# naman1618/Distributed-Inference-with-PyTorch-and-LiteLLM

Measured on AMD Instinct MI355X. Metric: fine-tune tokens/sec (whole node) Llama-3.1-70B DDP at 1/2/4/8 MI355X, higher is better.
Workload: dtype bf16; 1 GPU; model=Llama-3.1-70B, global_batch=2, seq_len=2048, parallelism=dp1, finetune=lora r=16 alpha=32.0 on q,k,v,o,gate,up,down; frozen bf16 base, micro_batch=2, grad_accum=1, activation_checkpointing=False, optimizer=fused AdamW (HIP), grad clip 1.0, grad_reduce_dtype=bf16

## Files before the change

### csrc/kernels/lora.hip

```cpp
#include "bindings.h"
#include "common.h"
#include <stdlib.h>
#include <string.h>

namespace mx {

namespace {

typedef __bf16 lbf16x8_t __attribute__((ext_vector_type(8)));
typedef __attribute__((address_space(1))) const void* lgptr_t;
typedef __attribute__((address_space(3))) void* llptr_t;

__device__ __forceinline__ f32x4 lmfma(const u16x8& a, const u16x8& b, const f32x4& c) {
  return __builtin_amdgcn_mfma_f32_16x16x32_bf16(__builtin_bit_cast(lbf16x8_t, a), __builtin_bit_cast(lbf16x8_t, b),
                                                 c, 0, 0, 0);
}

constexpr int kRS = 68;
constexpr int kMaxTiles = 16384;

__device__ unsigned int g_xwt_cnt[kMaxTiles];
__device__ unsigned int g_xtg_cnt[kMaxTiles];

__device__ __forceinline__ bool arrive_last(unsigned int* cnt, int S, int* s_flag) {
// ... 58 lines not shown
#pragma unroll
  for (int i = 0; i < 4; ++i)
#pragma unroll
    for (int j = 0; j < 4; ++j) acc[i][j] = f32x4{0.f, 0.f, 0.f, 0.f};

  auto load = [&](int b, u16x8(&xr)[4][2], u16x8(&vr)[4][2]) {
    const int k0 = b * 64;
#pragma unroll
    for (int i = 0; i < 4; ++i)
#pragma unroll
      for (int p = 0; p < 2; ++p) {
        xr[i][p] = *reinterpret_cast<const u16x8*>(xp + i * xrb + k0 + 8 * p);
        vr[i][p] = *reinterpret_cast<const u16x8*>(vp + i * vcb + k0 + 8 * p);
      }
  };
  auto comp = [&](const u16x8(&xr)[4][2], const u16x8(&vr)[4][2]) {
#pragma unroll
    for (int p = 0; p < 2; ++p)
#pragma unroll
      for (int i = 0; i < 4; ++i)
#pragma unroll
        for (int j = 0; j < 4; ++j) acc[i][j] = lmfma(xr[i][p], vr[j][p], acc[i][j]);
  };
  u16x8 xA[4][2], vA[4][2], xB[4][2], vB[4][2];
  int b = b0;
  if (b < b1) load(b, xA, vA);
  for (; b + 1 < b1; b += 2) {
    load(b + 1, xB, vB);
    __builtin_amdgcn_sched_barrier(0);
    comp(xA, vA);
    __builtin_amdgcn_sched_barrier(0);
    load(min(b + 2, b1 - 1), xA, vA);
    __builtin_amdgcn_sched_barrier(0);
    comp(xB, vB);
    __builtin_amdgcn_sched_barrier(0);
  }
  if (b < b1) comp(xA, vA);
  float* rw = red[w];
#pragma unroll
  for (int i = 0; i < 4; ++i)
#pragma unroll
    for (int j = 0; j < 4; ++j)
#pragma unroll
      for (int e = 0; e < 4; ++e) rw[(16 * i + 4 * g + e) * kRS + 16 * j + c] = acc[i][j][e];
  __syncthreads();
  float4 v[4];
#pragma unroll
  for (int q = 0; q < 4; ++q) {
    const int e4 = tid + 256 * q, row = e4 >> 4, col = (e4 & 15) * 4;
    float4 s = *reinterpret_cast<const float4*>(&red[0][row * kRS + col]);
#pragma unroll
    for (int ww = 1; ww < 4; ++ww) {
      const float4 t = *reinterpret_cast<const float4*>(&red[ww][row * kRS + col]);
      s.x += t.x, s.y += t.y, s.z += t.z, s.w += t.w;
    }
    v[q] = s;
  }
  if (S > 1) {
    float* wp = ws + ((int64_t)split * mtiles + mt) * 4096;
#pragma unroll
    for (int q = 0; q < 4; ++q) reinterpret_cast<float4*>(wp)[tid + 256 * q] = v[q];
    if (!fused_red) return;
    if (!arrive_last(&g_xwt_cnt[mt], S, &s_last)) return;
#pragma unroll
    for (int q = 0; q < 4; ++q) {
      float4 s = reinterpret_cast<const float4*>(ws + (int64_t)mt * 4096)[tid + 256 * q];
      for (int sp = 1; sp < S; ++sp) {
        const float4 t = reinterpret_cast<const float4*>(ws + ((int64_t)sp * mtiles + mt) * 4096)[tid + 256 * q];
        s.x += t.x, s.y += t.y, s.z += t.z, s.w += t.w;
      }
      v[q] = s;
    }
  }
#pragma unroll
  for (int q = 0; q < 4; ++q) {
    const int e4 = tid + 256 * q, row = e4 >> 4, col = (e4 & 15) * 4;
    uint2 o;
    o.x = pack_bf16x2(alpha * v[q].x, alpha * v[q].y);
    o.y = pack_bf16x2(alpha * v[q].z, alpha * v[q].w);
    *reinterpret_cast<uint2*>(out + (int64_t)(mt * 64 + row) * ldo + col) = o;
  }
}

__global__ void __launch_bounds__(256, 1) lora_xwt_lds_kernel(const uint16_t* __restrict__ X, int64_t ldx,
                                                              const uint16_t* __restrict__ V, int64_t ldv,
                                                              uint16_t* __restrict__ out, int64_t ldo,
                                                              float* __restrict__ ws, int M, int K, int S,
                                                              float alpha, int fused_red) {
  constexpr int TB = 8192, STG = 16384, WREG = 2 * STG;
  __shared__ __attribute__((aligned(16))) char smem[4 * WREG + 16];
  int* s_last = reinterpret_cast<int*>(smem + 4 * WREG);
  const int mtiles = M >> 6, mt = blockIdx.x, split = blockIdx.y;
  const int tid = threadIdx.x, lane = tid & 63, c = lane & 15, g = lane >> 4;
  const int w = __builtin_amdgcn_readfirstlane(tid >> 6);
  const int nb = K >> 6, nw = S * 4, gw = split * 4 + w;
  const int b0 = (int)((int64_t)gw * nb / nw), b1 = (int)((int64_t)(gw + 1) * nb / nw);
  char* wreg = smem + w * WREG;
  const uint32_t wbase = lds_addr(wreg);
  const int lrow = lane >> 3, sch = (lane & 7) ^ lrow;
  const uint16_t* xsrc = X + (int64_t)(mt * 64 + lrow) * ldx + 8 * sch;
  const uint16_t* vsrc = V + (int64_t)lrow * ldv + 8 * sch;
  auto issue = [&](int b, int s) {
    const int k0 = b * 64;
    char* xs = wreg + s * STG;
#pragma unroll
    for (int q = 0; q < 8; ++q)
      __builtin_amdgcn_global_load_lds((lgptr_t)(xsrc + (int64_t)(8 * q) * ldx + k0), (llptr_t)(xs + q * 1024), 16,
                                       0, 0);
#pragma unroll
    for (int q = 0; q < 8; ++q)
      __builtin_amdgcn_global_load_lds((lgptr_t)(vsrc + (int64_t)(8 * q) * ldv + k0), (llptr_t)(xs + TB + q * 1024),
                                       16, 0, 0);
  };
  const uint32_t rb0 = wbase + c * 128 + 16 * (g ^ (c & 7));
  const uint32_t rb1 = wbase + c * 128 + 16 * ((g ^ (c & 7)) ^ 4);

  f32x4 acc[4][4];
#pragma unroll
  for (int i = 0; i < 4; ++i)
#pragma unroll
    for (int j = 0; j < 4; ++j) acc[i][j] = f32x4{0.f, 0.f, 0.f, 0.f};

  auto block = [&](auto SC, int b) {
    constexpr int s = decltype(SC)::value;
    if (b + 1 < b1) asm volatile("s_waitcnt vmcnt(16)" ::: "memory");
    else asm volatile("s_waitcnt vmcnt(0)" ::: "memory");
    u16x8 xa[2][4], va[2][4];
#pragma unroll
    for (int i = 0; i < 4; ++i) {
      xa[0][i] = rd128_off(rb0, s * STG + i * 2048);
      xa[1][i] = rd128_off(rb1, s * STG + i * 2048);
      va[0][i] = rd128_off(rb0, s * STG + TB + i * 2048);
      va[1][i] = rd128_off(rb1, s * STG + TB + i * 2048);
    }
    lds_wait();
    __builtin_amdgcn_sched_barrier(0);
#pragma unroll
    for (int i = 0; i < 4; ++i) {
      pin(xa[0][i]), pin(xa[1][i]), pin(va[0][i]), pin(va[1][i]);
    }
    if (b + 2 < b1) issue(b + 2, s);
#pragma unroll
    for (int ks = 0; ks < 2; ++ks)
#pragma unroll
      for (int i = 0; i < 4; ++i)
#pragma unroll
        for (int j = 0; j < 4; ++j) acc[i][j] = lmfma(xa[ks][i], va[ks][j], acc[i][j]);
  };
  if (b0 < b1) issue(b0, 0);
  if (b0 + 1 < b1) issue(b0 + 1, 1);
  for (int b = b0; b < b1; b += 2) {
    block(std::integral_constant<int, 0>{}, b);
    if (b + 1 < b1) block(std::integral_constant<int, 1>{}, b + 1);
  }
  float* rw = reinterpret_cast<float*>(wreg);
#pragma unroll
  for (int i = 0; i < 4; ++i)
#pragma unroll
    for (int j = 0; j < 4; ++j)
#pragma unroll
      for (int e = 0; e < 4; ++e) rw[(16 * i + 4 * g + e) * kRS + 16 * j + c] = acc[i][j][e];
  __syncthreads();
  float4 v[4];
#pragma unroll
  for (int q = 0; q < 4; ++q) {
    const int e4 = tid + 256 * q, row = e4 >> 4, col = (e4 & 15) * 4;
    float4 s = *reinterpret_cast<const float4*>(reinterpret_cast<const float*>(smem) + row * kRS + col);
#pragma unroll
    for (int ww = 1; ww < 4; ++ww) {
      const float4 t = *reinterpret_cast<const float4*>(reinterpret_cast<const float*>(smem + ww * WREG) +
                                                        row * kRS + col);
      s.x += t.x, s.y += t.y, s.z += t.z, s.w += t.w;
    }
    v[q] = s;
  }
  if (S > 1) {
    float* wp = ws + ((int64_t)split * mtiles + mt) * 4096;
    if (!fused_red) {
#pragma unroll
      for (int q = 0; q < 4; ++q) reinterpret_cast<float4*>(wp)[tid + 256 * q] = v[q];
      return;
    }
#pragma unroll
    for (int q = 0; q < 4; ++q) st4_sc1(wp + 4 * (tid + 256 * q), v[q]);
    if (!arrive_last_sc1(&g_xwt_cnt[mt], S, s_last)) return;
#pragma unroll
    for (int q = 0; q < 4; ++q) {
      float4 s = ld4_sc1(ws + (int64_t)mt * 4096 + 4 * (tid + 256 * q));
      for (int sp = 1; sp < S; ++sp) {
        const float4 t = ld4_sc1(ws + ((int64_t)sp * mtiles + mt) * 4096 + 4 * (tid + 256 * q));
        s.x += t.x, s.y += t.y, s.z += t.z, s.w += t.w;
      }
      v[q] = s;
    }
  }
#pragma unroll
  for (int q = 0; q < 4; ++q) {
    const int e4 = tid + 256 * q, row = e4 >> 4, col = (e4 & 15) * 4;
    uint2 o;
    o.x = pack_bf16x2(alpha * v[q].x, alpha * v[q].y);
    o.y = pack_bf16x2(alpha * v[q].z, alpha * v[q].w);
    *reinterpret_cast<uint2*>(out + (int64_t)(mt * 64 + row) * ldo + col) = o;
  }
}

__global__ void __launch_bounds__(256) lora_xwt_reduce_kernel(const float* __restrict__ ws, int S, int mtiles,
                                                              uint16_t* __restrict__ out, int64_t ldo, float alpha,
                                                              int qpw) {
  const int per = 4 / qpw;
  const int mt = blockIdx.x / per, tid = threadIdx.x;
  for (int q = (blockIdx.x % per) * qpw; q < (blockIdx.x % per + 1) * qpw; ++q) {
    const int e4 = tid + 256 * q, row = e4 >> 4, col = (e4 & 15) * 4;
    float4 s = reinterpret_cast<const float4*>(ws + (int64_t)mt * 4096)[e4];
    for (int sp = 1; sp < S; ++sp) {
      const float4 t = reinterpret_cast<const float4*>(ws + ((int64_t)sp * mtiles + mt) * 4096)[e4];
      s.x += t.x, s.y += t.y, s.z += t.z, s.w += t.w;
    }
    uint2 o;
    o.x = pack_bf16x2(alpha * s.x, alpha * s.y);
    o.y = pack_bf16x2(alpha * s.z, alpha * s.w);
    *reinterpret_cast<uint2*>(out + (int64_t)(mt * 64 + row) * ldo + col) = o;
  }
}

struct XtgProb {
  const uint16_t* X;
  const uint16_t* G;
  uint16_t* out;
  int64_t ldx, ldg, os_n, os_j;
  int Nx, jb0, JB, tile0;
};
constexpr int kMaxProb = 8;
struct XtgArgs {
  XtgProb p[kMaxProb];
  int np, T, S, ntiles;
  float alpha;
  int accumulate;
  int fused_red;
  int narrow3;
  int wt;
};

__device__ __forceinline__ int xsw(int row) { return (((row >> 1) & 1) << 2) | (((row >> 2) & 1) << 1); }

__global__ void __launch_bounds__(256, 1) lora_xtg_kernel(const XtgArgs a, float* __restrict__ ws) {
  constexpr int XB = 8192, STG = 16384, WREG = 2 * STG;
  __shared__ __attribute__((aligned(16))) char smem[4 * WREG];
  __shared__ int s_last;
  const int tid = threadIdx.x, lane = tid & 63, c = lane & 15, g = lane >> 4;
  const int w = __builtin_amdgcn_readfirstlane(tid >> 6);
  const int tile = a.wt ? blockIdx.x * 4 + w : blockIdx.x, split = blockIdx.y;
  if (a.wt && tile >= a.ntiles) return;
  XtgProb P = a.p[0];
#pragma unroll
  for (int i = 1; i < kMaxProb; ++i)
    if (i < a.np && tile >= a.p[i].tile0) P = a.p[i];
  const int n0 = (tile - P.tile0) * 64;
  const bool wide = P.JB > 1;
  const int JB = P.JB;
  const int qq = c >> 2, pp = c & 3;
  const int nblk = a.T >> 6, nw = a.wt ? a.S : a.S * 4, gw = a.wt ? split : split * 4 + w;
  const int b0 = (int)((int64_t)gw * nblk / nw), b1 = (int)((int64_t)(gw + 1) * nblk / nw);
  char* wreg = smem + w * WREG;
  const uint32_t wbase = lds_addr(wreg);

  const int xrow = lane >> 3, xch = (lane & 7) ^ xsw(lane >> 3);
  const uint16_t* xsrc = P.X + (int64_t)xrow * P.ldx + n0 + 8 * xch;
  const uint16_t* gsrc = wide ? P.G + (int64_t)xrow * P.ldg + 16 * P.jb0 + 8 * xch
                              : P.G + (int64_t)(lane >> 1) * P.ldg + 16 * P.jb0 + 8 * (lane & 1);
  auto issue = [&](int b, int s) {
    const int64_t t0 = (int64_t)b * 64;
    char* xs = wreg + s * STG;
#pragma unroll
    for (int q = 0; q < 8; ++q)
      __builtin_amdgcn_global_load_lds((lgptr_t)(xsrc + (t0 + 8 * q) * P.ldx), (llptr_t)(xs + q * 1024), 16, 0, 0);
    if (wide) {
#pragma unroll
      for (int q = 0; q < 8; ++q)
        __builtin_amdgcn_global_load_lds((lgptr_t)(gsrc + (t0 + 8 * q) * P.ldg), (llptr_t)(xs + XB + q * 1024), 16, 0,
                                         0);
    } else {
#pragma unroll
      for (int q = 0; q < 2; ++q)
        __builtin_amdgcn_global_load_lds((lgptr_t)(gsrc + (t0 + 32 * q) * P.ldg), (llptr_t)(xs + XB + q * 1024), 16,
                                         0, 0);
    }
  };
  const int fl = xsw(4 * g + qq);
  uint32_t xb[4];
#pragma unroll
  for (int i = 0; i < 4; ++i) xb[i] = wbase + (4 * g + qq) * 128 + 16 * ((2 * i + (pp >> 1)) ^ fl) + 8 * (pp & 1);
  const uint32_t gnb = wbase + XB + (4 * g + qq) * 32 + 8 * pp;

  f32x4 acc[4][4];
#pragma unroll
  for (int i = 0; i < 4; ++i)
#pragma unroll
    for (int j = 0; j < 4; ++j) acc[i][j] = f32x4{0.f, 0.f, 0.f, 0.f};

  auto block = [&](auto SC, int b) {
    constexpr int s = decltype(SC)::value;
    if (b + 1 < b1) {
      if (wide) asm volatile("s_waitcnt vmcnt(16)" ::: "memory");
      else asm volatile("s_waitcnt vmcnt(10)" ::: "memory");
// ... 393 lines not shown
    }
  }
}

}

using namespace mx;

static int lora_env(const char* name, int dflt);

static int swiglu_lora_rbw(int T) {
  int rbw = lora_env("MXLLM_SWIGLU_LORA_RBW", 2);
  rbw = rbw >= 4 ? 4 : (rbw >= 2 ? 2 : 1);
  while (rbw > 1 && (T / 16) % rbw) rbw >>= 1;
  return rbw;
}

static int swiglu_lora_splits(int T, int F) {
  const int tiles = F / 128, rbs = T / (16 * swiglu_lora_rbw(T));
  int cs = lora_env("MXLLM_SWIGLU_LORA_CS", 0);
  if (cs <= 0) cs = (512 + rbs - 1) / rbs;
  cs = cs < 1 ? 1 : cs;
  cs = cs > tiles ? tiles : cs;
  return cs > 32 ? 32 : cs;
}

extern "C" int64_t mx_swiglu_lora_ws(int T, int F, int nrb) {
  if (T <= 0 || F < 128) return 0;
  return (int64_t)swiglu_lora_splits(T, F) * T * 16 * nrb;
}

extern "C" int mx_swiglu_lora(int bwd, const uint16_t* gu, const uint16_t* dm, uint16_t* out, int64_t ldo,
                              const uint16_t* V, int64_t ldv, int nrb, int pad, float alpha, float* ws, int T, int F,
                              hipStream_t stream) {
  if (T <= 0) return 0;
  if (T % 16 || F % 128 || nrb < 1 || nrb > 4 || pad < 16 * nrb || pad % 8 || ldo % 8 || ldv % 8 ||
      ldo < (bwd ? 2 * (int64_t)F : F) + pad || ((uintptr_t)gu | (uintptr_t)out | (uintptr_t)V) % 16 ||
      (bwd && (!dm || (uintptr_t)dm % 16)))
    return (int)hipErrorInvalidValue;
  const int CS = swiglu_lora_splits(T, F), RBW = swiglu_lora_rbw(T);
  const dim3 grid(T / (16 * RBW), CS);
#define MX_SL_R(B, N, R) swiglu_lora_kernel<B, N, R><<<grid, 256, 0, stream>>>(gu, dm, out, ldo, V, ldv, ws, F, CS)
#define MX_SL(B, N)                                 \
  do {                                              \
    if (RBW == 4) MX_SL_R(B, N, 4);                 \
    else if (RBW == 2) MX_SL_R(B, N, 2);            \
    else MX_SL_R(B, N, 1);                          \
  } while (0)
  if (bwd) {
    switch (nrb) { case 1: MX_SL(true, 1); break; case 2: MX_SL(true, 2); break;
                   case 3: MX_SL(true, 3); break; default: MX_SL(true, 4); break; }
  } else {
    switch (nrb) { case 1: MX_SL(false, 1); break; case 2: MX_SL(false, 2); break;
                   case 3: MX_SL(false, 3); break; default: MX_SL(false, 4); break; }
  }
#undef MX_SL
#undef MX_SL_R
  swiglu_lora_reduce_kernel<<<T / 16, 256, 0, stream>>>(ws, CS, 16 * nrb, pad, out + (bwd ? 2 * (int64_t)F : F), ldo,
                                                        alpha);
  return (int)hipGetLastError();
}

static int lora_env(const char* name, int dflt) {
  const char* v = getenv(name);
  return v && *v ? atoi(v) : dflt;
}
static int lora_splits(int tiles, int blocks, int smax) {
  if (tiles <= 0) return 1;
  const int target = lora_env("MXLLM_LORA_WGS", 256);
  int S = (target + tiles - 1) / tiles;
  S = S < 1 ? 1 : (S > smax ? smax : S);
  while (S > 1 && blocks / (4 * S) < 2) --S;
  return S;
}

static bool xtg_wave_tiles(int ntiles) {
  return lora_env("MXLLM_LORA_XTG_WT", 1) == 1 && ntiles >= lora_env("MXLLM_LORA_XTG_WT_MIN", 1024);
}

static int xwt_mode() {
  const char* kv = getenv("MXLLM_LORA_XWT");
  if (kv && !strcmp(kv, "reg")) return 2;
  if (kv && !strcmp(kv, "tile")) return 0;
  return 1;
}
static bool xwt_tile_ok(const void* X, int64_t ldx, const void* V, int64_t ldv, int M, int K, int rows) {
  return xwt_mode() == 0 && M % 16 == 0 && K % 128 == 0 && rows > 0 && rows <= 64 && ldx % 8 == 0 &&
         ldv % 8 == 0 && (uintptr_t)X % 16 == 0 && (uintptr_t)V % 16 == 0;
}
static int xwt_rbw(int M) { return M % 64 == 0 ? 4 : (M % 32 == 0 ? 2 : 1); }
static int xwt_tile_splits(int M, int K) {
  const int groups = M / (16 * xwt_rbw(M)), tiles = K / 128;
  int cs = lora_env("MXLLM_LORA_XWT_CS", 0);
  if (cs <= 0) cs = (512 + groups - 1) / groups;
  cs = cs < 1 ? 1 : cs;
  return cs > tiles ? tiles : cs;
}

extern "C" int64_t mx_lora_xwt_ws(int M, int K, int rows) {
  const int S = M >= 64 && K >= 64 ? lora_splits(M / 64, K / 64, 16) : 1;
  const int64_t dma = S > 1 ? (int64_t)S * (M / 64) * 4096 : 0;
  if (rows > 0 && rows <= 64 && M % 16 == 0 && K % 128 == 0 && xwt_mode() == 0) {
    const int64_t tile = (int64_t)xwt_tile_splits(M, K) * M * 16 * ((rows + 15) / 16);
    return tile > dma ? tile : dma;
  }
  return dma;
}
extern "C" int64_t mx_lora_xtg_ws(int ntiles, int T) {
  if (xtg_wave_tiles(ntiles)) return 0;
  const int S = lora_splits(ntiles, T / 64, 8);
  return S > 1 ? (int64_t)S * ntiles * 4096 : 0;
}

extern "C" int mx_lora_xwt(const uint16_t* X, int64_t ldx, const uint16_t* V, int64_t ldv, int Vrows, uint16_t* out,
                           int64_t ldo, float* ws, int M, int K, float alpha, int rows, hipStream_t stream) {
  if (M <= 0) return 0;
  if (xwt_tile_ok(X, ldx, V, ldv, M, K, rows) && rows <= Vrows && ldo % 4 == 0) {
    const int nrb = (rows + 15) / 16, rbw = xwt_rbw(M), CS = xwt_tile_splits(M, K);
    const dim3 grid(M / (16 * rbw), CS);
#define MX_XT(N, R) lora_xwt_tile_kernel<N, R><<<grid, 256, 0, stream>>>(X, ldx, V, ldv, ws, K, CS)
#define MX_XT_N(R)                                  \
  switch (nrb) {                                    \
    case 1: MX_XT(1, R); break;                     \
    case 2: MX_XT(2, R); break;                     \
    case 3: MX_XT(3, R); break;                     \
    default: MX_XT(4, R); break;                    \
  }
    if (rbw == 4) { MX_XT_N(4) } else if (rbw == 2) { MX_XT_N(2) } else { MX_XT_N(1) }
#undef MX_XT_N
#undef MX_XT
    swiglu_lora_reduce_kernel<<<M / 16, 256, 0, stream>>>(ws, CS, 16 * nrb, Vrows, out, ldo, alpha);
    return (int)hipGetLastError();
  }
  if (M % 64 || K % 64 || Vrows % 64 || M / 64 > kMaxTiles) return (int)hipErrorInvalidValue;
  const int mtiles = M / 64, S = lora_splits(mtiles, K / 64, 16);
  const int fused = lora_env("MXLLM_LORA_FUSED_RED", 0);
  const bool lds = xwt_mode() != 2 && ((uintptr_t)X % 16 == 0) && ((uintptr_t)V % 16 == 0) && ldx % 8 == 0 &&
                   ldv % 8 == 0;
  for (int c0 = 0; c0 < Vrows; c0 += 64) {
    if (lds)
      lora_xwt_lds_kernel<<<dim3(mtiles, S), 256, 0, stream>>>(X, ldx, V + (int64_t)c0 * ldv, ldv, out + c0, ldo, ws,
                                                               M, K, S, alpha, fused);
    else
      lora_xwt_kernel<<<dim3(mtiles, S), 256, 0, stream>>>(X, ldx, V + (int64_t)c0 * ldv, ldv, out + c0, ldo, ws, M,
                                                           K, S, alpha, fused);
    if (S > 1 && !fused) {
      const int qpw = lora_env("MXLLM_LORA_XWT_RED_ROWS", 16) >= 64 ? 4 : 1;
      lora_xwt_reduce_kernel<<<(4 / qpw) * mtiles, 256, 0, stream>>>(ws, S, mtiles, out + c0, ldo, alpha, qpw);
    }
  }
  return (int)hipGetLastError();
}

extern "C" int mx_lora_xtg(const int64_t* desc, int np, int T, float alpha, int accumulate, float* ws,
                           hipStream_t stream) {
  if (np <= 0 || np > kMaxProb || T % 64) return (int)hipErrorInvalidValue;
  if (T == 0) return 0;
  XtgArgs a{};
  int ntiles = 0;
  for (int i = 0; i < np; ++i) {
    const int64_t* d = desc + i * 10;
    XtgProb& p = a.p[i];
    p.X = reinterpret_cast<const uint16_t*>(d[0]);
    p.G = reinterpret_cast<const uint16_t*>(d[1]);
    p.out = reinterpret_cast<uint16_t*>(d[2]);
    p.ldx = d[3], p.ldg = d[4], p.os_n = d[5], p.os_j = d[6];
    p.Nx = (int)d[7], p.jb0 = (int)d[8], p.JB = (int)d[9];
    if (p.Nx <= 0 || p.Nx % 64 || p.JB < 1 || p.JB > 4) return (int)hipErrorInvalidValue;
    p.tile0 = ntiles;
    ntiles += p.Nx / 64;
  }
  if (ntiles > kMaxTiles) return (int)hipErrorInvalidValue;
  a.np = np, a.T = T, a.ntiles = ntiles, a.alpha = alpha;
  a.wt = xtg_wave_tiles(ntiles);
  a.S = a.wt ? 1 : lora_splits(ntiles, T / 64, 8);
  a.accumulate = accumulate;
  a.fused_red = a.wt ? 0 : lora_env("MXLLM_LORA_FUSED_RED", 0);
  a.narrow3 = lora_env("MXLLM_LORA_XTG_STAGES", 3) == 3;
  lora_xtg_kernel<<<dim3(a.wt ? (ntiles + 3) / 4 : ntiles, a.S), 256, 0, stream>>>(a, ws);
  if (a.S > 1 && !a.fused_red) lora_xtg_reduce_kernel<<<ntiles, 256, 0, stream>>>(a, ws);
  return (int)hipGetLastError();
}
```

### mxllm/ops/linear.py

```python
from __future__ import annotations

import math
import os
from typing import Sequence

import torch
import torch.nn.functional as F

from ..parallel.grad_ready import direct_grad, direct_grad32, mark_ready
from . import gemm
from ._ext import native, use_native


class _LoRALinearFn(torch.autograd.Function):
    @staticmethod
    def forward(ctx, x, w, a, b, scaling, splits, r):
        x2 = x.reshape(-1, x.shape[-1])
        t = torch.matmul(x2, a.t())
        y = torch.empty(x2.shape[0], w.shape[0], dtype=x.dtype, device=x.device)
        y.addmm_(t, b.t(), beta=0.0, alpha=scaling)
        y.addmm_(x2, w.t())
        ctx.save_for_backward(x2, w, a, b, t)
        ctx.scaling, ctx.splits, ctx.r, ctx.xshape = scaling, tuple(splits), r, x.shape
        return y.view(*x.shape[:-1], w.shape[0])

    @staticmethod
    def backward(ctx, dy):
        x2, w, a, b, t = ctx.saved_tensors
        s, r = ctx.scaling, ctx.r
        dy2 = dy.reshape(-1, dy.shape[-1])
        g = torch.empty(dy2.shape[0], a.shape[0], dtype=dy2.dtype, device=dy2.device)
        g.addmm_(dy2, b, beta=0.0, alpha=s)
        ga, gb = direct_grad(a) if ctx.needs_input_grad[2] else None, direct_grad(b) if ctx.needs_input_grad[3] else None
        da = db = None
        if ctx.needs_input_grad[2]:
            if ga is not None:
                ga.addmm_(g.t(), x2)
                mark_ready(a)
            else:
                da = torch.matmul(g.t(), x2)
        if ctx.needs_input_grad[3]:
            tgt = gb if gb is not None else torch.zeros_like(b)
            off = 0
            for i, n_i in enumerate(ctx.splits):
                tgt[off:off + n_i, i * r:(i + 1) * r].addmm_(dy2[:, off:off + n_i].t(), t[:, i * r:(i + 1) * r],
                                                            beta=1.0 if gb is not None else 0.0, alpha=s)
                off += n_i
            if gb is not None:
                mark_ready(b)
            else:
                db = tgt
        dx = torch.matmul(g, a)
        dx.addmm_(dy2, w)
        return dx.view(ctx.xshape), None, da, db, None, None, None


def _padded_rows(t: torch.Tensor, pad: int) -> torch.Tensor | None:
    if t.dim() != 2 or t.stride(1) != 1 or t.stride(0) != t.shape[1] + pad:
        return None
    st = t.untyped_storage()
    need = (t.storage_offset() + t.shape[0] * t.stride(0)) * t.element_size()
    if st.nbytes() < need:
        return None
    full = torch.empty(0, dtype=t.dtype, device=t.device)
    full.set_(st, t.storage_offset(), (t.shape[0], t.shape[1] + pad), (t.stride(0), 1))
    return full


def _augment(t: torch.Tensor, pad: int) -> torch.Tensor:
    full = _padded_rows(t, pad)
    if full is None:
        full = torch.empty(t.shape[0], t.shape[1] + pad, dtype=t.dtype, device=t.device)
        full[:, :t.shape[1]].copy_(t)
    return full


_LORA_KERNELS = os.environ.get("MXLLM_LORA_KERNELS", "1") != "0"


def _lora_native(x2: torch.Tensor, N: int, K: int, splits, r: int, wbt) -> bool:
    return (_LORA_KERNELS and wbt is not None and use_native(x2) and x2.shape[0] % 64 == 0 and K % 64 == 0 and r % 16 == 0
            and r <= 64 and all(n % 64 == 0 for n in splits) and x2.dtype == torch.bfloat16)


def _lora_aug_backward(ctx, xa, wbuf, dy, dy_tail: bool, need_a: bool, need_b: bool):
    N, K, s, splits, r, pad, xshape, nat, tr = ctx.dims
    R = r * len(splits)
    dy2 = dy.reshape(-1, N)
    dya = _padded_rows(dy2, pad) if dy_tail else None
    if dya is None:
        dya = _augment(dy2, pad)
        if nat:
            native().lora_xwt(dy2, ctx.wbt, dya[:, N:], s, len(splits) * r)
        else:
            bmat = wbuf[K:, :N].t() if tr else wbuf[:N, K:]
            dya[:, N:].addmm_(dy2, bmat, beta=0.0, alpha=s)
    g = dya[:, N:N + R]
    x2, st = xa[:, :K], xa[:, K:K + R]
    da = db = None
    ga = direct_grad(ctx.lora_a) if need_a else None
    gb = direct_grad(ctx.lora_b) if need_b else None
    if nat and need_a and need_b:
        acc = ga is not None and gb is not None
        tga = ga if acc else torch.empty(R, K, dtype=dy2.dtype, device=dy2.device)
        tgb = gb if acc else torch.zeros(N, R, dtype=dy2.dtype, device=dy2.device)
        native().lora_grads(x2, dy2, dya[:, N:], xa[:, K:], tga, tgb, list(splits), r, acc)
        if acc:
            mark_ready(ctx.lora_a)
            mark_ready(ctx.lora_b)
        else:
            da, db = tga, tgb
    else:
        if need_a:
            if ga is not None:
                ga.addmm_(g.t(), x2)
                mark_ready(ctx.lora_a)
            else:
                da = torch.mm(g.t(), x2)
        if need_b:
            tgt = gb if gb is not None else torch.zeros(N, R, dtype=dy2.dtype, device=dy2.device)
            off = 0
            for i, n_i in enumerate(splits):
                tgt[off:off + n_i, i * r:(i + 1) * r].addmm_(dy2[:, off:off + n_i].t(), st[:, i * r:(i + 1) * r],
                                                            beta=1.0 if gb is not None else 0.0)
                off += n_i
            if gb is not None:
                mark_ready(ctx.lora_b)
            else:
                db = tgt
    if tr:
        dx = gemm.mm("tn", dya, wbuf[:K, :])
    elif ctx.wxt is not None:
        dx = gemm.mm("tn", dya, ctx.wxt)
    else:
        dx = gemm.mm("nn", dya, wbuf[:, :K])
    return dx.view(xshape), da, db


class _LoRAAugFn(torch.autograd.Function):

    @staticmethod
    def forward(ctx, x, a, b, wbuf, scaling, splits, r, pad, wbt, wxt=None, wa=None, x_tail=False, dy_tail=False):
        tr = wa is not None
        if tr:
            K, N = wbuf.shape[0] - pad, wbuf.shape[1] - pad
        else:
            N, K = wbuf.shape[0] - pad, wbuf.shape[1] - pad
        x2 = x.reshape(-1, K)
        nat = _lora_native(x2, N, K, splits, r, wbt)
        xa = _padded_rows(x2, pad) if x_tail else None
        if xa is None:
            xa = _augment(x2, pad)
            amat = wa if tr else wbuf[N:, :K]
            if nat:
                native().lora_xwt(x2, amat, xa[:, K:], scaling, a.shape[0])
            else:
                xa[:, K:].addmm_(x2, amat.t(), beta=0.0, alpha=scaling)
        y = gemm.mm("nn", xa, wbuf[:, :N]) if tr else gemm.mm("tn", xa, wbuf[:N, :])
        ctx.save_for_backward(xa, wbuf)
        ctx.lora_a, ctx.lora_b, ctx.wbt, ctx.wxt = a, b, wbt, wxt
        ctx.dims = (N, K, scaling, tuple(splits), r, pad, x.shape, nat, tr)
        ctx.dy_tail = dy_tail
        return y.view(*x.shape[:-1], N)

    @staticmethod
    def backward(ctx, dy):
        xa, wbuf = ctx.saved_tensors
        dx, da, db = _lora_aug_backward(ctx, xa, wbuf, dy, ctx.dy_tail, ctx.needs_input_grad[1],
                                        ctx.needs_input_grad[2])
        return dx, da, db, None, None, None, None, None, None, None, None, None, None


def lora_linear_aug(x: torch.Tensor, a: torch.Tensor, b: torch.Tensor, wbuf: torch.Tensor, splits: Sequence[int],
                    scaling: float, pad: int, wbt: torch.Tensor | None = None,
                    wxt: torch.Tensor | None = None, wa: torch.Tensor | None = None,
                    x_tail: bool = False, dy_tail: bool = False) -> torch.Tensor:
    r = a.shape[0] // len(splits)
    return _LoRAAugFn.apply(x, a, b, wbuf, scaling, tuple(splits), r, pad, wbt, wxt, wa, bool(x_tail), bool(dy_tail))


_LORA_QKV_ROPE = os.environ.get("MXLLM_LORA_QKV_ROPE", "1") != "0"


def lora_qkv_attention_at(x: torch.Tensor, lin, B: int, S: int, Hq: int, Hkv: int, D: int) -> int:
    if not (_LORA_QKV_ROPE and lin.lora_r > 0 and lin.augmented() and not lin.transposed and D == 128
            and S % 256 == 0 and use_native(x) and x.dtype == torch.bfloat16 and not gemm.deterministic()):
        return 0
    N, K, pad = sum(lin.splits), lin.in_features, lin.pad
    x2 = x.reshape(-1, x.shape[-1])
    if N != (Hq + 2 * Hkv) * D or x2.shape[0] != B * S or x2.shape[1] != K:
        return 0
    xa = _padded_rows(x2, pad)
    if xa is None or not gemm.schedule("tn", B * S, N, K + pad, torch.bfloat16):
        return 0
    at = gemm.tail_at("tn", B * S, N, K + pad, torch.bfloat16)
    return at if at > 0 and gemm.g8_rope_takes(xa, lin.wbuf[:N, :], S, Hq, Hkv, at) else 0


def _lora_aug_input(x2, a, wbuf, amat, scaling, N, K, pad, nat):
    xa = _augment(x2, pad)
    if nat:
        native().lora_xwt(x2, amat, xa[:, K:], scaling, a.shape[0])
    else:
        xa[:, K:].addmm_(x2, amat.t(), beta=0.0, alpha=scaling)
    return xa


class _LoRAQKVAttnFn(torch.autograd.Function):

    @staticmethod
    def forward(ctx, x, a, b, wbuf, scaling, splits, r, pad, wbt, wxt, cos, sin, B, S, Hq, Hkv, D, causal, out_pad,
                at):
        N, K = wbuf.shape[0] - pad, wbuf.shape[1] - pad
        x2 = x.reshape(-1, K)
        nat = _lora_native(x2, N, K, splits, r, wbt)
        xa = _lora_aug_input(x2, a, wbuf, wbuf[N:, :K], scaling, N, K, pad, nat)
        ops = native()
        q = torch.empty(B, Hq, S, D, dtype=x.dtype, device=x.device)
        k = torch.empty(B, Hkv, S, D, dtype=x.dtype, device=x.device)
        v = torch.empty_like(k)
        if not ops.gemm8_rope_tail(xa, wbuf[:N, :], cos, sin, B, S, Hq, Hkv, q, k, v, at):
            q, k, v = ops.rope_split(gemm.mm("tn", xa, wbuf[:N, :]), cos, sin, B, S, Hq, Hkv, D)
        o, lse = ops.attn_fwd(q, k, v, causal, 1.0 / math.sqrt(D), out_pad)
        ctx.save_for_backward(xa, wbuf, q, k, v, o, lse, cos, sin)
        ctx.lora_a, ctx.lora_b, ctx.wbt, ctx.wxt = a, b, wbt, wxt
        ctx.dims = (N, K, scaling, tuple(splits), r, pad, x.shape, nat, False)
        ctx.causal = causal
        return o.view(B * S, Hq * D)

    @staticmethod
    def backward(ctx, do):
        from .attention import backward_dqkv

        xa, wbuf, q, k, v, o, lse, cos, sin = ctx.saved_tensors
        pad = ctx.dims[5]
        dqkv = backward_dqkv(do, q, k, v, o, lse, cos, sin, ctx.causal, pad)
        del q, k, v, o, lse
        dx, da, db = _lora_aug_backward(ctx, xa, wbuf, dqkv, False, ctx.needs_input_grad[1], ctx.needs_input_grad[2])
        return (dx, da, db) + (None,) * 17


def lora_qkv_attention(x: torch.Tensor, lin, cos: torch.Tensor, sin: torch.Tensor, B: int, S: int, Hq: int,
                       Hkv: int, D: int, at: int, causal: bool = True, out_pad: int = 0) -> torch.Tensor:
    r = lin.lora_a.shape[0] // len(lin.splits)
    return _LoRAQKVAttnFn.apply(x, lin.lora_a, lin.lora_b, lin.wbuf, lin.scaling, tuple(lin.splits), r, lin.pad,
                                lin.wbt, getattr(lin, "wxt", None), cos, sin, B, S, Hq, Hkv, D, causal, out_pad, at)


def transpose2d(t: torch.Tensor, scale: torch.Tensor | None = None) -> torch.Tensor:
    if use_native(t):
        if t.stride(-1) != 1:
            t = t.contiguous()
        return native().transpose2d(t, scale)
    out = t.t().contiguous()
    return out if scale is None else (out * scale.to(out.dtype))


def copy2d_plan(pairs) -> tuple[list[list[int]], int]:
    rows, total = [], 0
    for s, d in pairs:
        assert s.shape == d.shape and s.dim() == 2 and s.element_size() == 2 and d.element_size() == 2
        r, c = s.shape
        rows.append([s.data_ptr(), d.data_ptr(), r, c, s.stride(0), d.stride(0), total, s.stride(1), d.stride(1)])
        if s.stride(1) == 1 and d.stride(0) == 1 and d.stride(1) != 1:
            total += ((r + 63) // 64) * ((c + 63) // 64)
        else:
            total += (r * c + 4095) // 4096
    return rows, total


_DW_TN = os.environ.get("MXLLM_DW_TN", "1") != "0"


def weight_grad_(out: torch.Tensor | None, dy: torch.Tensor, x: torch.Tensor, beta: float = 1.0,
                 dy_scale: torch.Tensor | None = None) -> torch.Tensor:
    f32 = out is not None and out.dtype == torch.float32 and dy.dtype != torch.float32
    if use_native(dy) and dy.dtype == torch.bfloat16 and x.dtype == torch.bfloat16:
        odt = out.dtype if out is not None else dy.dtype
        if gemm.want("tt", dy.shape[1], x.shape[1], dy.shape[0], odt):
            sc = None if dy_scale is None else dy_scale.reshape(1).float()
            return gemm.mm("tt", dy, x, out=out, beta=beta if out is not None else 0.0, alpha_t=sc,
                           out_dtype=odt)
    if _DW_TN and use_native(dy) and dy.dtype == torch.bfloat16 and x.dtype == torch.bfloat16:
        xt = transpose2d(x)
        dyt = transpose2d(dy, None if dy_scale is None else dy_scale.reshape(1).float())
        if out is None:
            return torch.mm(dyt, xt.t())
        if f32:
            return torch.ops.aten.addmm.dtype_out(out, dyt, xt.t(), torch.float32, beta=beta, out=out)
        return out.addmm_(dyt, xt.t(), beta=beta)
    if dy_scale is not None:
        dy = dy * dy_scale.to(dy.dtype)
    if out is None:
        return torch.mm(dy.t(), x)
    if f32:
        if dy.is_cuda:
            return torch.ops.aten.addmm.dtype_out(out, dy.t(), x, torch.float32, beta=beta, out=out)
        return out.addmm_(dy.t().float(), x.float(), beta=beta)
    return out.addmm_(dy.t(), x, beta=beta)


def param_weight_grad(wp: torch.Tensor | None, dy: torch.Tensor, x: torch.Tensor,
                      dy_scale: torch.Tensor | None = None) -> torch.Tensor | None:
    g = direct_grad(wp) if wp is not None else None
    if g is None and wp is not None:
        g = direct_grad32(wp)
    if g is None:
        return weight_grad_(None, dy, x, dy_scale=dy_scale)
    fresh = getattr(wp, "_mx_grad_fresh", False)
    armed = getattr(wp, "_mx_sq_done", None)
    sq = getattr(wp, "_mx_sq", None) if fresh and armed is False else None
    if sq is not None and g.dtype == dy.dtype == x.dtype == torch.bfloat16 and gemm.mm_sq(
            "tt", dy, x, g, sq, None if dy_scale is None else dy_scale.reshape(1).float()):
        wp._mx_sq_done = True
    else:
        if armed is True:
            wp._mx_sq_done = "dirty"
        weight_grad_(g, dy, x, beta=0.0 if fresh else 1.0, dy_scale=dy_scale)
    if fresh:
        wp._mx_grad_fresh = False
    mark_ready(wp)
# ... 189 lines not shown
```

Before: 4815 tokens/s.

## Size LoRA X·Wᵀ tiles to the rank and skip unneeded input-gradient GEMMs

The LDS-staged X·Aᵀ kernel is templated on output column blocks, pipeline stages and row tiles, so a rank-16 LoRA computes only 16 columns instead of padding to 64. It also gets a 3-stage prefetch and optionally 32-row tiles, and the padding columns are zero-filled. The split-K workspace layout and the reduce kernel change to match the narrower tiles. Separately, the backward pass skips computing dx when the input does not need a gradient, for example at the first layer. This cuts MFMA work and loads for low ranks, at the cost of more kernel variants and a new default mode.

```diff
diff --git a/csrc/kernels/lora.hip b/csrc/kernels/lora.hip
--- a/csrc/kernels/lora.hip
+++ b/csrc/kernels/lora.hip
@@ -164,15 +164,20 @@
   }
 }
 
-__global__ void __launch_bounds__(256, 1) lora_xwt_lds_kernel(const uint16_t* __restrict__ X, int64_t ldx,
-                                                              const uint16_t* __restrict__ V, int64_t ldv,
-                                                              uint16_t* __restrict__ out, int64_t ldo,
-                                                              float* __restrict__ ws, int M, int K, int S,
-                                                              float alpha, int fused_red) {
-  constexpr int TB = 8192, STG = 16384, WREG = 2 * STG;
-  __shared__ __attribute__((aligned(16))) char smem[4 * WREG + 16];
-  int* s_last = reinterpret_cast<int*>(smem + 4 * WREG);
-  const int mtiles = M >> 6, mt = blockIdx.x, split = blockIdx.y;
+template <int NRB, int NST, int MR>
+__global__ void __launch_bounds__(256, MR == 4 ? 1 : 2)
+    lora_xwt_lds_kernel(const uint16_t* __restrict__ X, int64_t ldx, const uint16_t* __restrict__ V, int64_t ldv,
+                        uint16_t* __restrict__ out, int64_t ldo, float* __restrict__ ws, int M, int K, int S,
+                        float alpha, int fused_red) {
+  constexpr int TR = 16 * MR, NC = 16 * NRB;
+  constexpr int TB = 2048 * MR, STG = TB + 2048 * NRB;
+  constexpr int WREG = NST * STG;
+  constexpr int P = 2 * (MR + NRB);
+  static_assert(WREG >= TR * kRS * 4 + 16, "the wave's region also holds its reduction image");
+  static_assert((NST - 1) * P < 64, "vmcnt is a 6-bit counter");
+  __shared__ __attribute__((aligned(16))) char smem[4 * WREG];
+  int* s_last = reinterpret_cast<int*>(smem + 4 * WREG - 16);
+  const int mt = blockIdx.x, split = blockIdx.y;
   const int tid = threadIdx.x, lane = tid & 63, c = lane & 15, g = lane >> 4;
   const int w = __builtin_amdgcn_readfirstlane(tid >> 6);
   const int nb = K >> 6, nw = S * 4, gw = split * 4 + w;
@@ -180,73 +185,82 @@
   char* wreg = smem + w * WREG;
   const uint32_t wbase = lds_addr(wreg);
   const int lrow = lane >> 3, sch = (lane & 7) ^ lrow;
-  const uint16_t* xsrc = X + (int64_t)(mt * 64 + lrow) * ldx + 8 * sch;
+  const uint16_t* xsrc = X + (int64_t)(mt * TR + lrow) * ldx + 8 * sch;
   const uint16_t* vsrc = V + (int64_t)lrow * ldv + 8 * sch;
   auto issue = [&](int b, int s) {
     const int k0 = b * 64;
     char* xs = wreg + s * STG;
 #pragma unroll
-    for (int q = 0; q < 8; ++q)
+    for (int q = 0; q < 2 * MR; ++q)
       __builtin_amdgcn_global_load_lds((lgptr_t)(xsrc + (int64_t)(8 * q) * ldx + k0), (llptr_t)(xs + q * 1024), 16,
                                        0, 0);
 #pragma unroll
-    for (int q = 0; q < 8; ++q)
+    for (int q = 0; q < 2 * NRB; ++q)
       __builtin_amdgcn_global_load_lds((lgptr_t)(vsrc + (int64_t)(8 * q) * ldv + k0), (llptr_t)(xs + TB + q * 1024),
                                        16, 0, 0);
   };
   const uint32_t rb0 = wbase + c * 128 + 16 * (g ^ (c & 7));
   const uint32_t rb1 = wbase + c * 128 + 16 * ((g ^ (c & 7)) ^ 4);
 
-  f32x4 acc[4][4];
-#pragma unroll
-  for (int i = 0; i < 4; ++i)
-#pragma unroll
-    for (int j = 0; j < 4; ++j) acc[i][j] = f32x4{0.f, 0.f, 0.f, 0.f};
+  f32x4 acc[MR][NRB];
+#pragma unroll
+  for (int i = 0; i < MR; ++i)
+#pragma unroll
+    for (int j = 0; j < NRB; ++j) acc[i][j] = f32x4{0.f, 0.f, 0.f, 0.f};
 
   auto block = [&](auto SC, int b) {
     constexpr int s = decltype(SC)::value;
-    if (b + 1 < b1) asm volatile("s_waitcnt vmcnt(16)" ::: "memory");
+    if (b + NST - 1 < b1) asm volatile("s_waitcnt vmcnt(%0)" ::"n"((NST - 1) * P) : "memory");
+    else if (NST == 3 && b + 1 < b1) asm volatile("s_waitcnt vmcnt(%0)" ::"n"(P) : "memory");
     else asm volatile("s_waitcnt vmcnt(0)" ::: "memory");
-    u16x8 xa[2][4], va[2][4];
-#pragma unroll
-    for (int i = 0; i < 4; ++i) {
+    u16x8 xa[2][MR], va[2][NRB];
+#pragma unroll
+    for (int i = 0; i < MR; ++i) {
       xa[0][i] = rd128_off(rb0, s * STG + i * 2048);
       xa[1][i] = rd128_off(rb1, s * STG + i * 2048);
-      va[0][i] = rd128_off(rb0, s * STG + TB + i * 2048);
-      va[1][i] = rd128_off(rb1, s * STG + TB + i * 2048);
+    }
+#pragma unroll
+    for (int j = 0; j < NRB; ++j) {
+      va[0][j] = rd128_off(rb0, s * STG + TB + j * 2048);
+      va[1][j] = rd128_off(rb1, s * STG + TB + j * 2048);
     }
     lds_wait();
     __builtin_amdgcn_sched_barrier(0);
 #pragma unroll
-    for (int i = 0; i < 4; ++i) {
-      pin(xa[0][i]), pin(xa[1][i]), pin(va[0][i]), pin(va[1][i]);
-    }
-    if (b + 2 < b1) issue(b + 2, s);
+    for (int i = 0; i < MR; ++i) pin(xa[0][i]), pin(xa[1][i]);
+#pragma unroll
+    for (int j = 0; j < NRB; ++j) pin(va[0][j]), pin(va[1][j]);
+    if (b + NST < b1) issue(b + NST, s);
 #pragma unroll
     for (int ks = 0; ks < 2; ++ks)
 #pragma unroll
-      for (int i = 0; i < 4; ++i)
-#pragma unroll
-        for (int j = 0; j < 4; ++j) acc[i][j] = lmfma(xa[ks][i], va[ks][j], acc[i][j]);
+      for (int i = 0; i < MR; ++i)
+#pragma unroll
+        for (int j = 0; j < NRB; ++j) acc[i][j] = lmfma(xa[ks][i], va[ks][j], acc[i][j]);
   };
-  if (b0 < b1) issue(b0, 0);
-  if (b0 + 1 < b1) issue(b0 + 1, 1);
-  for (int b = b0; b < b1; b += 2) {
+#pragma unroll
+  for (int s = 0; s < NST; ++s)
+    if (b0 + s < b1) issue(b0 + s, s);
+  for (int b = b0; b < b1; b += NST) {
     block(std::integral_constant<int, 0>{}, b);
     if (b + 1 < b1) block(std::integral_constant<int, 1>{}, b + 1);
+    if constexpr (NST == 3)
+      if (b + 2 < b1) block(std::integral_constant<int, 2>{}, b + 2);
   }
   float* rw = reinterpret_cast<float*>(wreg);
 #pragma unroll
-  for (int i = 0; i < 4; ++i)
-#pragma unroll
-    for (int j = 0; j < 4; ++j)
+  for (int i = 0; i < MR; ++i)
+#pragma unroll
+    for (int j = 0; j < NRB; ++j)
 #pragma unroll
       for (int e = 0; e < 4; ++e) rw[(16 * i + 4 * g + e) * kRS + 16 * j + c] = acc[i][j][e];
   __syncthreads();
-  float4 v[4];
-#pragma unroll
-  for (int q = 0; q < 4; ++q) {
-    const int e4 = tid + 256 * q, row = e4 >> 4, col = (e4 & 15) * 4;
+  constexpr int NF4 = TR * NC / 4, NQ = (NF4 + 255) / 256, F4R = NC / 4;
+  float4 v[NQ];
+#pragma unroll
+  for (int q = 0; q < NQ; ++q) {
+    const int e4 = tid + 256 * q, row = e4 / F4R, col = (e4 % F4R) * 4;
+    if (e4 >= NF4) continue;
     float4 s = *reinterpret_cast<const float4*>(reinterpret_cast<const float*>(smem) + row * kRS + col);
 #pragma unroll
     for (int ww = 1; ww < 4; ++ww) {
@@ -257,51 +271,70 @@
     v[q] = s;
   }
   if (S > 1) {
-    float* wp = ws + ((int64_t)split * mtiles + mt) * 4096;
+    const int64_t sstride = (int64_t)M * NC;
+    float* wp = ws + (int64_t)split * sstride + (int64_t)mt * (TR * NC);
     if (!fused_red) {
 #pragma unroll
-      for (int q = 0; q < 4; ++q) reinterpret_cast<float4*>(wp)[tid + 256 * q] = v[q];
+      for (int q = 0; q < NQ; ++q)
+        if (tid + 256 * q < NF4) reinterpret_cast<float4*>(wp)[tid + 256 * q] = v[q];
       return;
     }
 #pragma unroll
-    for (int q = 0; q < 4; ++q) st4_sc1(wp + 4 * (tid + 256 * q), v[q]);
+    for (int q = 0; q < NQ; ++q)
+      if (tid + 256 * q < NF4) st4_sc1(wp + 4 * (tid + 256 * q), v[q]);
     if (!arrive_last_sc1(&g_xwt_cnt[mt], S, s_last)) return;
 #pragma unroll
-    for (int q = 0; q < 4; ++q) {
-      float4 s = ld4_sc1(ws + (int64_t)mt * 4096 + 4 * (tid + 256 * q));
+    for (int q = 0; q < NQ; ++q) {
+      if (tid + 256 * q >= NF4) continue;
+      const float* rp = ws + (int64_t)mt * (TR * NC) + 4 * (tid + 256 * q);
+      float4 s = ld4_sc1(rp);
       for (int sp = 1; sp < S; ++sp) {
-        const float4 t = ld4_sc1(ws + ((int64_t)sp * mtiles + mt) * 4096 + 4 * (tid + 256 * q));
+        const float4 t = ld4_sc1(rp + sp * sstride);
         s.x += t.x, s.y += t.y, s.z += t.z, s.w += t.w;
       }
       v[q] = s;
     }
   }
 #pragma unroll
-  for (int q = 0; q < 4; ++q) {
-    const int e4 = tid + 256 * q, row = e4 >> 4, col = (e4 & 15) * 4;
+  for (int q = 0; q < NQ; ++q) {
+    const int e4 = tid + 256 * q, row = e4 / F4R, col = (e4 % F4R) * 4;
+    if (e4 >= NF4) continue;
     uint2 o;
     o.x = pack_bf16x2(alpha * v[q].x, alpha * v[q].y);
     o.y = pack_bf16x2(alpha * v[q].z, alpha * v[q].w);
-    *reinterpret_cast<uint2*>(out + (int64_t)(mt * 64 + row) * ldo + col) = o;
+    *reinterpret_cast<uint2*>(out + (int64_t)(mt * TR + row) * ldo + col) = o;
+  }
+  if constexpr (NRB < 4) {
+    constexpr int ZR = (64 - NC) / 4;
+    for (int z = tid; z < TR * ZR; z += 256)
+      *reinterpret_cast<uint2*>(out + (int64_t)(mt * TR + z / ZR) * ldo + NC + 4 * (z % ZR)) = uint2{0u, 0u};
   }
 }
 
 __global__ void __launch_bounds__(256) lora_xwt_reduce_kernel(const float* __restrict__ ws, int S, int mtiles,
                                                               uint16_t* __restrict__ out, int64_t ldo, float alpha,
-                                                              int qpw) {
+                                                              int qpw, int nrb) {
   const int per = 4 / qpw;
   const int mt = blockIdx.x / per, tid = threadIdx.x;
+  const int f4r = 4 * nrb, nc = 16 * nrb, zr = 16 - f4r;
+  const int64_t sstride = (int64_t)mtiles * 64 * nc;
   for (int q = (blockIdx.x % per) * qpw; q < (blockIdx.x % per + 1) * qpw; ++q) {
-    const int e4 = tid + 256 * q, row = e4 >> 4, col = (e4 & 15) * 4;
-    float4 s = reinterpret_cast<const float4*>(ws + (int64_t)mt * 4096)[e4];
-    for (int sp = 1; sp < S; ++sp) {
-      const float4 t = reinterpret_cast<const float4*>(ws + ((int64_t)sp * mtiles + mt) * 4096)[e4];
-      s.x += t.x, s.y += t.y, s.z += t.z, s.w += t.w;
-    }
-    uint2 o;
-    o.x = pack_bf16x2(alpha * s.x, alpha * s.y);
-    o.y = pack_bf16x2(alpha * s.z, alpha * s.w);
-    *reinterpret_cast<uint2*>(out + (int64_t)(mt * 64 + row) * ldo + col) = o;
+    if (tid < 16 * f4r) {
+      const int row = 16 * q + tid / f4r, col = (tid % f4r) * 4;
+      const float* rp = ws + ((int64_t)mt * 64 + row) * nc + col;
+      float4 s = *reinterpret_cast<const float4*>(rp);
+      for (int sp = 1; sp < S; ++sp) {
+        const float4 t = *reinterpret_cast<const float4*>(rp + sp * sstride);
+        s.x += t.x, s.y += t.y, s.z += t.z, s.w += t.w;
+      }
+      uint2 o;
+      o.x = pack_bf16x2(alpha * s.x, alpha * s.y);
+      o.y = pack_bf16x2(alpha * s.z, alpha * s.w);
+      *reinterpret_cast<uint2*>(out + (int64_t)(mt * 64 + row) * ldo + col) = o;
+    } else {
+      const int z = tid - 16 * f4r;
+      *reinterpret_cast<uint2*>(out + (int64_t)(mt * 64 + 16 * q + z / zr) * ldo + nc + 4 * (z % zr)) = uint2{0u, 0u};
+    }
   }
 }
 
@@ -861,7 +894,8 @@
   const char* kv = getenv("MXLLM_LORA_XWT");
   if (kv && !strcmp(kv, "reg")) return 2;
   if (kv && !strcmp(kv, "tile")) return 0;
-  return 1;
+  if (kv && !strcmp(kv, "lds")) return 1;
+  return 3;
 }
 static bool xwt_tile_ok(const void* X, int64_t ldx, const void* V, int64_t ldv, int M, int K, int rows) {
   return xwt_mode() == 0 && M % 16 == 0 && K % 128 == 0 && rows > 0 && rows <= 64 && ldx % 8 == 0 &&
@@ -913,21 +947,42 @@
   }
   if (M % 64 || K % 64 || Vrows % 64 || M / 64 > kMaxTiles) return (int)hipErrorInvalidValue;
   const int mtiles = M / 64, S = lora_splits(mtiles, K / 64, 16);
+  const int mode = xwt_mode();
+  const bool lds = mode != 2 && ((uintptr_t)X % 16 == 0) && ((uintptr_t)V % 16 == 0) && ldx % 8 == 0 &&
+                   ldv % 8 == 0;
+  const bool rowsf = lds && mode == 3 && rows > 0 && rows <= 64 && Vrows == 64;
+  const int nrb = rowsf ? (rows + 15) / 16 : 4;
+  const bool mt32 = rowsf && nrb <= 3 && M / 32 <= kMaxTiles && lora_env("MXLLM_LORA_XWT_MT", 64) == 32;
+  const bool st3 = rowsf && lora_env("MXLLM_LORA_XWT_STAGES", 3) == 3 && nrb <= (mt32 ? 1 : 2);
   const int fused = lora_env("MXLLM_LORA_FUSED_RED", 0);
-  const bool lds = xwt_mode() != 2 && ((uintptr_t)X % 16 == 0) && ((uintptr_t)V % 16 == 0) && ldx % 8 == 0 &&
-                   ldv % 8 == 0;
+  const int xfused = rowsf ? lora_env("MXLLM_LORA_XWT_FUSED", fused) : fused;
+#define MX_XL(N, ST, R)                                                                                          \
+  lora_xwt_lds_kernel<N, ST, R><<<dim3(M / (16 * R), S), 256, 0, stream>>>(X, ldx, V + (int64_t)c0 * ldv, ldv,    \
+                                                                           out + c0, ldo, ws, M, K, S, alpha, xfused)
   for (int c0 = 0; c0 < Vrows; c0 += 64) {
-    if (lds)
-      lora_xwt_lds_kernel<<<dim3(mtiles, S), 256, 0, stream>>>(X, ldx, V + (int64_t)c0 * ldv, ldv, out + c0, ldo, ws,
-                                                               M, K, S, alpha, fused);
-    else
+    if (lds && mt32) {
+      switch (nrb) {
+        case 1: if (st3) MX_XL(1, 3, 2); else MX_XL(1, 2, 2); break;
+        case 2: MX_XL(2, 2, 2); break;
+        default: MX_XL(3, 2, 2); break;
+      }
+    } else if (lds) {
+      switch (nrb) {
+        case 1: if (st3) MX_XL(1, 3, 4); else MX_XL(1, 2, 4); break;
+        case 2: if (st3) MX_XL(2, 3, 4); else MX_XL(2, 2, 4); break;
+        case 3: MX_XL(3, 2, 4); break;
+        default: MX_XL(4, 2, 4); break;
+      }
+    } else {
       lora_xwt_kernel<<<dim3(mtiles, S), 256, 0, stream>>>(X, ldx, V + (int64_t)c0 * ldv, ldv, out + c0, ldo, ws, M,
                                                            K, S, alpha, fused);
-    if (S > 1 && !fused) {
+    }
+    if (S > 1 && !(lds ? xfused : fused)) {
       const int qpw = lora_env("MXLLM_LORA_XWT_RED_ROWS", 16) >= 64 ? 4 : 1;
-      lora_xwt_reduce_kernel<<<(4 / qpw) * mtiles, 256, 0, stream>>>(ws, S, mtiles, out + c0, ldo, alpha, qpw);
-    }
-  }
+      lora_xwt_reduce_kernel<<<(4 / qpw) * mtiles, 256, 0, stream>>>(ws, S, mtiles, out + c0, ldo, alpha, qpw, nrb);
+    }
+  }
+#undef MX_XL
   return (int)hipGetLastError();
 }
 
diff --git a/mxllm/ops/linear.py b/mxllm/ops/linear.py
--- a/mxllm/ops/linear.py
+++ b/mxllm/ops/linear.py
@@ -50,6 +50,8 @@
                 mark_ready(b)
             else:
                 db = tgt
+        if not ctx.needs_input_grad[0]:
+            return None, None, da, db, None, None, None
         dx = torch.matmul(g, a)
         dx.addmm_(dy2, w)
         return dx.view(ctx.xshape), None, da, db, None, None, None
@@ -83,7 +85,7 @@
             and r <= 64 and all(n % 64 == 0 for n in splits) and x2.dtype == torch.bfloat16)
 
 
-def _lora_aug_backward(ctx, xa, wbuf, dy, dy_tail: bool, need_a: bool, need_b: bool):
+def _lora_aug_backward(ctx, xa, wbuf, dy, dy_tail: bool, need_a: bool, need_b: bool, need_x: bool = True):
     N, K, s, splits, r, pad, xshape, nat, tr = ctx.dims
     R = r * len(splits)
     dy2 = dy.reshape(-1, N)
@@ -128,6 +130,8 @@
                 mark_ready(ctx.lora_b)
             else:
                 db = tgt
+    if not need_x:
+        return None, da, db
     if tr:
         dx = gemm.mm("tn", dya, wbuf[:K, :])
     elif ctx.wxt is not None:
@@ -167,7 +171,7 @@
     def backward(ctx, dy):
         xa, wbuf = ctx.saved_tensors
         dx, da, db = _lora_aug_backward(ctx, xa, wbuf, dy, ctx.dy_tail, ctx.needs_input_grad[1],
-                                        ctx.needs_input_grad[2])
+                                        ctx.needs_input_grad[2], ctx.needs_input_grad[0])
         return dx, da, db, None, None, None, None, None, None, None, None, None, None
 
 
@@ -236,7 +240,8 @@
         pad = ctx.dims[5]
         dqkv = backward_dqkv(do, q, k, v, o, lse, cos, sin, ctx.causal, pad)
         del q, k, v, o, lse
-        dx, da, db = _lora_aug_backward(ctx, xa, wbuf, dqkv, False, ctx.needs_input_grad[1], ctx.needs_input_grad[2])
+        dx, da, db = _lora_aug_backward(ctx, xa, wbuf, dqkv, False, ctx.needs_input_grad[1], ctx.needs_input_grad[2],
+                                        ctx.needs_input_grad[0])
         return (dx, da, db) + (None,) * 17
 
 
```

Result: no change. 4822 tokens/s, median of 4 (+0.1%).
